# sp-uhh/sgmse

Measured on AMD Instinct MI355X. Metric: utterances/sec, SGMSE+ NCSN++ PC N=30 (reverse_diffusion + ALD, 60 NFE), 16 kHz 4 s utterances, higher is better.
Workload: dtype f32 (fp16x2-split products, fp32 accumulate); 1 GPU; BASELINE configs[1]: ncsnpp (65.6M params) PC sampler N=30, batch=32 x 4 s @16 kHz per GPU, hipGraph-captured step; batch_per_gpu=32, F=256, T=512, nfe=60, sampler=pc, parallelism=utterance-sharded x1 (weights broadcast once over RCCL)

## Files before the change

sgmse_amd/csrc/kernels_conv_split.h:

```cpp
#pragma once
#include "kernels_conv.h"

#ifndef SGMSE_SPLIT_FENCE
#define SGMSE_SPLIT_FENCE 0
#endif

namespace sgmse {

struct SplitB3 {
  static constexpr int NS = 3;
  static constexpr int NP = 6;
  static constexpr int PX_V = 7;
  static constexpr bool SCALED = false;
  __device__ static constexpr int pa(int k) { return k == 0 ? 2 : (k == 2 || k == 3) ? 1 : 0; }
  __device__ static constexpr int pb(int k) { return k == 1 ? 2 : (k == 2 || k == 4) ? 1 : 0; }
  __device__ static __forceinline__ void split(float x, uint32_t (&t)[3]) {
    const uint32_t xb = __builtin_bit_cast(uint32_t, x);
    const uint32_t hi = xb & 0xffff0000u;
    const float r1 = x - __builtin_bit_cast(float, hi);
    const uint32_t mid = __builtin_bit_cast(uint32_t, r1) & 0xffff0000u;
    const float r2 = r1 - __builtin_bit_cast(float, mid);
    t[0] = hi >> 16; t[1] = mid >> 16; t[2] = __builtin_bit_cast(uint32_t, r2) >> 16;
  }
  __device__ static __forceinline__ void split2(float x0, float x1, uint32_t (&d)[3]) {
    uint32_t a[3], b[3];
    split(x0, a); split(x1, b);
#pragma unroll
    for (int s = 0; s < 3; ++s) d[s] = a[s] | (b[s] << 16);
  }
  __device__ static __forceinline__ f32x16 mfma(u32x4 a, u32x4 b, f32x16 c) { return mfma_32x32x16_bf16(a, b, c); }
};

struct SplitH2 {
  static constexpr int NS = 2;
  static constexpr int NP = 3;
  static constexpr int PX_V = 5;
  static constexpr bool SCALED = true;
  __device__ static constexpr int pa(int k) { return k == 0 ? 1 : 0; }
  __device__ static constexpr int pb(int k) { return k == 1 ? 1 : 0; }
  __device__ static __forceinline__ void split(float x, uint32_t (&t)[2]) {
    const uint32_t hi = drt_f32_to_f16(x);
    const float r = x - drt_f16_to_f32(hi);
    t[0] = hi; t[1] = drt_f32_to_f16(r);
  }
  __device__ static __forceinline__ void split2(float x0, float x1, uint32_t (&d)[2]) {
    const uint32_t hi = drt_f32x2_to_f16x2(x0, x1);
    d[0] = hi; d[1] = drt_f32x2_to_f16x2(drt_sub_f16_lo(x0, hi), drt_sub_f16_hi(x1, hi));
  }
  __device__ static __forceinline__ f32x16 mfma(u32x4 a, u32x4 b, f32x16 c) { return mfma_32x32x16_f16(a, b, c); }
};

template <int ROWS_>
struct ConvSplitGeom {
  static constexpr int KC = 16, ROWS = ROWS_, TROWS = ROWS_ + 2, TCOLS = 34;
  static constexpr int NITEM = TROWS * TCOLS * 2;
  static constexpr int NIT = (NITEM + 255) / 256;
};

struct PackSplitArgs { const float* src; uint32_t* dst; int cin, cout; size_t total; const float* co_scale; int taps; };
__global__ __launch_bounds__(256) void split_co_scale_kernel(const float* src, int n_per_co, int cout, int cout_pad, float* inv_scale, float* scale) {
  const int co = blockIdx.x * 256 + threadIdx.x;
  if (co >= cout_pad) return;
  float m = 0.f;
  if (co < cout) for (int i = 0; i < n_per_co; ++i) m = fmaxf(m, fabsf(src[(size_t)co * n_per_co + i]));
  const float sc = co < cout ? h2_weight_scale(m) : 1.f;
  scale[co] = sc; inv_scale[co] = 1.f / sc;
}

__global__ __launch_bounds__(256) void absmax_kernel(const float* x, size_t n, float* out) {
  float m = 0.f;
  for (size_t i = (size_t)blockIdx.x * 256 + threadIdx.x; i < n; i += (size_t)gridDim.x * 256) m = fmaxf(m, fabsf(x[i]));
#pragma unroll
  for (int o = 32; o >= 1; o >>= 1) m = fmaxf(m, __shfl_xor(m, o));
  if ((threadIdx.x & 63) == 0) drt_atomic_max_nonneg(out, m);
}

template <class S>
__global__ __launch_bounds__(256) void pack_weights_split_kernel(PackSplitArgs p) {
  const size_t e = (size_t)blockIdx.x * 256 + threadIdx.x;
  if (e >= p.total) return;
  const int lane = (int)(e & 63);
  size_t r = e >> 6;
  const int w = (int)(r & 3); r >>= 2;
  const int split = (int)(r % S::NS); r /= S::NS;
  const int tap = (int)(r % p.taps); r /= p.taps;
  const int nst = p.cin / 16;
  const int st = (int)(r % nst);
  const int blk = (int)(r / nst);
  const int co = blk * 128 + w * 32 + (lane & 31);
  const int c0 = st * 16 + 8 * (lane >> 5);
  const float wscale = (S::SCALED && co < p.cout) ? p.co_scale[co] : 1.f;
  u32x4 o;
#pragma unroll
  for (int q = 0; q < 4; ++q) {
    uint32_t part[2];
#pragma unroll
    for (int h = 0; h < 2; ++h) {
      const int c = c0 + 2 * q + h;
      const float v = (co < p.cout ? p.src[((size_t)co * p.cin + c) * p.taps + tap] : 0.f) * wscale;
      uint32_t t[S::NS];
      S::split(v, t);
      uint32_t sel = t[0];
#pragma unroll
      for (int s = 1; s < S::NS; ++s) sel = split == s ? t[s] : sel;
      part[h] = sel;
    }
    o[q] = part[0] | (part[1] << 16);
  }
  reinterpret_cast<u32x4*>(p.dst)[e] = o;
}

template <class S>
inline size_t packed_split_frags(int cin, int cout, int taps = 9) { return (size_t)((cout + 127) / 128) * (cin / 16) * taps * S::NS * 4 * 64; }
template <class S>
inline size_t packed_split_bytes(int cin, int cout, int taps = 9) { return packed_split_frags<S>(cin, cout, taps) * 16 + (size_t)((cout + 127) / 128) * 128 * 8; }

template <class S, int SHAPE = 0, int ACT = 1, int ABL = 0, int SC = 0, int CHK = 0>
__global__ __launch_bounds__(256, 2) void conv3x3_split_kernel(ConvArgs p) {
  static_assert(!CHK || (SHAPE == 2 && !SC), "chunked accumulation exists for the plain 4-row shape");
  constexpr bool THIN = SHAPE == 1;
  constexpr int ROWS = SHAPE == 2 ? 4 : 8;
  using C = ConvSplitGeom<ROWS>;
  constexpr int WCW = THIN ? 1 : 4;
  constexpr int FCW = THIN ? 1 : 4 / WCW;
  constexpr int FPW = THIN ? 2 : ROWS / (4 / WCW);
  using T = ConvTile<3, WCW, FCW, FPW, 1>;
  static_assert(T::CO_T == (THIN ? 32 : 128) && T::ROWS == ROWS, "tile");
  constexpr int NS = S::NS, PX_V = S::PX_V;
  constexpr int EPJ = 8 / FPW;
  constexpr int STAGE_V = C::TROWS * C::TCOLS * PX_V;
  constexpr int DUMMY_V = STAGE_V;
  __shared__ u32x4 s_in0[STAGE_V + NS];
  __shared__ u32x4 s_in1[STAGE_V + NS];
  constexpr int NCO = S::SCALED ? 4 : 2;
  __shared__ float s_co[512 * NCO];

  const int tid = threadIdx.x;
  if constexpr (ABL & 512) {
    __shared__ u32x4 s_pad[3072];
    if (p.ablate == 12345) s_pad[tid] = u32x4{0u, 0u, 0u, 0u};
  }
  unsigned long long* trace = nullptr;
  if constexpr (ABL & 64) {
    if (tid == 0 && p.trace) {
      trace = p.trace + 16 * (size_t)(blockIdx.y * gridDim.x + blockIdx.x);
      trace[0] = (unsigned long long)drt_hw_id() | ((unsigned long long)drt_xcc_id() << 32);
      trace[1] = drt_clock();
    }
  }
  const int Cin = p.C1 + p.C2;
  const int tiles_xg = (p.W + 31) >> 5;
  const int tiles_y = (p.H + ROWS - 1) / ROWS;
  int b, ty, tx;
  conv_tile_of(p, (int)blockIdx.x, (int)gridDim.x, tiles_xg, tiles_y, b, ty, tx);
  if (p.rag_w) { if (!conv_ragged_adjust(p, b, tx)) return; }
  const int H = p.H, W = p.W;
  const int tiles_x = (W + 31) >> 5;
  const int co_blk = blockIdx.y;
  const int x0 = tx * 32, y0 = ty * ROWS;
  float xb_raw = 0.f;
  if constexpr (S::SCALED) { if (p.xbound) xb_raw = p.xbound[b * kAmaxSpread + (tid & (kAmaxSpread - 1))]; }
  float csc[2], csh[2];
#pragma unroll
  for (int k = 0; k < 2; ++k) {
    const int c = tid + 256 * k;
    const bool ld = p.in_scale != nullptr && c < Cin;
    csc[k] = ld ? p.in_scale[b * Cin + (c < Cin ? c : 0)] : 1.f;
    csh[k] = ld ? p.in_shift[b * Cin + (c < Cin ? c : 0)] : 0.f;
  }
  const unsigned HW = (unsigned)H * (unsigned)W;

  const int wave = tid >> 6, lane = tid & 63, l31 = lane & 31, kg = lane >> 5;

  unsigned it_boff[C::NIT];
  int it_loff[C::NIT], it_g[C::NIT];
#pragma unroll
  for (int i = 0; i < C::NIT; ++i) {
    int it = tid + 256 * i;
    it = it < C::NITEM ? it : C::NITEM - 1;
    const int g = it / (C::TROWS * C::TCOLS);
    const int rem = it - g * (C::TROWS * C::TCOLS);
    const int r = rem / C::TCOLS, c = rem - r * C::TCOLS;
    const int gy = y0 - 1 + r, gx = x0 - 1 + c;
    const bool ok = gy >= 0 && gy < H && gx >= 0 && gx < W;
    const int loff = (r * C::TCOLS + c) * PX_V + g * NS;
    if (!ok) {
#pragma unroll
      for (int s = 0; s < NS; ++s) { s_in0[loff + s] = u32x4{0u, 0u, 0u, 0u}; s_in1[loff + s] = u32x4{0u, 0u, 0u, 0u}; }
    }
    it_boff[i] = ((unsigned)(8 * g) * HW + (ok ? (unsigned)(gy * W + gx) : 0u)) * 4u;
    it_loff[i] = ok ? loff : DUMMY_V;
    it_g[i] = g;
  }

  float rin[C::NIT][8];
  auto load_item = [&](int i, int c0) {
    const bool first = c0 < p.C1;
    const float* base = first ? p.src1 + ((size_t)b * p.C1 + c0) * HW : p.src2 + ((size_t)b * p.C2 + (c0 - p.C1)) * HW;
#pragma unroll
    for (int e = 0; e < 8; ++e)
      rin[i][e] = *reinterpret_cast<const float*>(reinterpret_cast<const char*>(base + (size_t)e * HW) + it_boff[i]);
  };
  auto produce = [&](float x, int ch) -> float {
    float o, u;
    if constexpr (NCO == 4) {
      const f32x4 co = reinterpret_cast<const f32x4*>(s_co)[ch];
      o = x * co[0] + co[1];
      u = x * co[2] + co[3];
    } else {
      o = x * s_co[2 * ch] + s_co[2 * ch + 1];
      u = o * -1.4426950408889634f;
    }
    if constexpr (ACT == 1) {
      if constexpr (ABL & 4) o = o * u;
      else o = o * __builtin_amdgcn_rcpf(1.0f + drt_exp2(u));
    }
    if (S::SCALED) o = fminf(fmaxf(o, -65504.f), 65504.f);
    return o;
  };
  auto store_item = [&](int i, int c0, u32x4* sbuf) {
    u32x4 v[NS];
#pragma unroll
    for (int q = 0; q < 4; ++q) {
      const int ch = c0 + 8 * it_g[i] + 2 * q;
      uint32_t d[NS];
      S::split2(produce(rin[i][2 * q], ch), produce(rin[i][2 * q + 1], ch + 1), d);
#pragma unroll
      for (int s = 0; s < NS; ++s) v[s][q] = d[s];
    }
#pragma unroll
    for (int s = 0; s < NS; ++s) sbuf[it_loff[i] + s] = v[s];
  };

  u32x4 pk[NS];
  float ev = 0.f;
  auto stage_elem = [&](int i, int e, int c0, const float (&raw)[C::NIT][8]) {
    const float o = produce(raw[i][e], c0 + 8 * it_g[i] + e);
    if ((e & 1) == 0) { ev = o; return; }
    uint32_t d[NS];
    S::split2(ev, o, d);
#pragma unroll
    for (int s = 0; s < NS; ++s) pk[s][e >> 1] = d[s];
  };
  auto flush_item = [&](int i, u32x4* sbuf) {
#pragma unroll
    for (int s = 0; s < NS; ++s) sbuf[it_loff[i] + s] = pk[s];
  };

  const int wc = THIN ? 0 : wave % WCW, wp = THIN ? wave : wave / WCW;
  const int nst = Cin / C::KC;
  int st0 = 0, st1 = nst;
  if constexpr (CHK) {
    if (gridDim.z > 1) { st0 = (int)blockIdx.z * p.kchunk_stages; st1 = st0 + p.kchunk_stages < nst ? st0 + p.kchunk_stages : nst; }
  }
  float acc_raw[(SC || CHK) ? 1 : FCW][16];
  if constexpr (!(SC || CHK)) {
#pragma unroll
    for (int i = 0; i < FCW; ++i) conv_acc_raw<T>(p, b, co_blk, wc * FCW + i, kg, acc_raw[i]);
  }
  float sc_m1 = 0.f, sc_m2 = 0.f;
  if constexpr (SC) {
    sc_m1 = p.sc_amax1[b * kAmaxSpread + (tid & (kAmaxSpread - 1))];
    if (p.sc_amax2) sc_m2 = p.sc_amax2[b * kAmaxSpread + (tid & (kAmaxSpread - 1))];
  } else {
#pragma unroll
    for (int i = 0; i < C::NIT; ++i) load_item(i, st0 * C::KC);
  }
  float kx = 1.f;
  if constexpr (S::SCALED) {
    if (p.xbound) {
#pragma unroll
      for (int o = 32; o >= 1; o >>= 1) xb_raw = fmaxf(xb_raw, __shfl_xor(xb_raw, o));
      kx = h2_weight_scale(xb_raw);
    }
  }
  const float inv_kx = 1.f / kx;
  {
    constexpr float nl2e = -1.4426950408889634f;
#pragma unroll
    for (int k = 0; k < 2; ++k) {
      const int c = tid + 256 * k;
      if (c < Cin) {
        if constexpr (NCO == 4) {
          f32x4 v;
          v[0] = csc[k] * kx; v[1] = csh[k] * kx; v[2] = csc[k] * nl2e; v[3] = csh[k] * nl2e;
          reinterpret_cast<f32x4*>(s_co)[c] = v;
        } else {
          s_co[2 * c] = csc[k] * kx; s_co[2 * c + 1] = csh[k] * kx;
        }
      }
    }
  }
  f32x16 acc[FCW][FPW];
#pragma unroll
  for (int i = 0; i < FCW; ++i) {
    float init[16];
    if constexpr (SC || CHK) {
#pragma unroll
      for (int r = 0; r < 16; ++r) init[r] = 0.f;
    } else {
      const int co_l = co_blk * T::CO_T + (wc * FCW + i) * 32 + 4 * kg;
#pragma unroll
      for (int r = 0; r < 16; ++r) init[r] = acc_raw[i][r] * (1.0f / (conv_as(p, co_l + (r & 3) + 8 * (r >> 2)) * inv_kx));
    }
#pragma unroll
    for (int j = 0; j < FPW; ++j)
#pragma unroll
      for (int r = 0; r < 16; ++r) acc[i][j][r] = init[r];
  }

  const u32x4* wblk = reinterpret_cast<const u32x4*>(p.w) + (size_t)co_blk * nst * 9 * NS * 4 * 64;
  const unsigned a_boff = (unsigned)((wc * FCW * 64 + lane) * 16);
  const bool a_real = !THIN || l31 < p.Cout;
  auto load_a = [&](int st, int tap, u32x4 (&a)[FCW][NS]) {
    const u32x4* q = wblk + (size_t)(st * 9 + tap) * NS * 4 * 64;
#pragma unroll
    for (int i = 0; i < FCW; ++i)
#pragma unroll
      for (int s = 0; s < NS; ++s) {
        if constexpr (THIN) {
          a[i][s] = u32x4{0u, 0u, 0u, 0u};
          if (a_real) a[i][s] = *reinterpret_cast<const u32x4*>(reinterpret_cast<const char*>(q + s * 4 * 64 + i * 64) + a_boff);
        } else {
          a[i][s] = *reinterpret_cast<const u32x4*>(reinterpret_cast<const char*>(q + s * 4 * 64 + i * 64) + a_boff);
        }
      }
  };
  const int b_lane = l31 * PX_V + kg * NS + wp * FPW * C::TCOLS * PX_V;

  u32x4 bq[2][NS];
  auto compute_tap = [&](const u32x4* sbuf, int tap, const u32x4 (&a)[FCW][NS], int item, int c0n, u32x4* nxt, const float (&raw)[C::NIT][8]) {
    const int dy = tap / 3, dx = tap - 3 * dy;
    const u32x4* sb = sbuf + b_lane + (dy * C::TCOLS + dx) * PX_V;
    if constexpr (!(ABL & 16)) {
#pragma unroll
      for (int s = 0; s < NS; ++s) bq[0][s] = sb[s];
    }
#pragma unroll
    for (int j = 0; j < FPW; ++j) {
      if constexpr (!(ABL & 16)) {
        if (j + 1 < FPW) {
          const u32x4* q = sb + (j + 1) * C::TCOLS * PX_V;
#pragma unroll
          for (int s = 0; s < NS; ++s) bq[(j + 1) & 1][s] = q[s];
        }
      }
      __builtin_amdgcn_sched_barrier(SGMSE_SPLIT_FENCE);
#pragma unroll
      for (int k = 0; k < S::NP; ++k)
#pragma unroll
        for (int i = 0; i < FCW; ++i) acc[i][j] = S::mfma(a[i][S::pa(k)], bq[j & 1][S::pb(k)], acc[i][j]);
      if (item >= 0) {
#pragma unroll
        for (int e = 0; e < EPJ; ++e) stage_elem(item, j * EPJ + e, c0n, raw);
        if (j == FPW - 1) flush_item(item, nxt);
      }
      __builtin_amdgcn_sched_barrier(SGMSE_SPLIT_FENCE);
    }
  };

  if constexpr (SC) {
    static_assert(S::SCALED && !THIN, "the folded shortcut exists for the fp16x2 full-block shapes");
    float m = fmaxf(sc_m1, sc_m2);
#pragma unroll
    for (int o = 32; o >= 1; o >>= 1) m = fmaxf(m, __shfl_xor(m, o));
    const float xs = h2_weight_scale(m);
    const int nsts = (p.sc_C1 + p.sc_C2) / C::KC;
    float rsc[C::NIT][8];
    auto load_sc = [&](int c0, float (&dst)[C::NIT][8]) {
      const bool first = c0 < p.sc_C1;
      const float* base = first ? p.sc_src1 + ((size_t)b * p.sc_C1 + c0) * HW : p.sc_src2 + ((size_t)b * p.sc_C2 + (c0 - p.sc_C1)) * HW;
#pragma unroll
      for (int i = 0; i < C::NIT; ++i)
#pragma unroll
        for (int e = 0; e < 8; ++e)
          dst[i][e] = *reinterpret_cast<const float*>(reinterpret_cast<const char*>(base + (size_t)e * HW) + it_boff[i]);
    };
    auto store_sc = [&](const float (&src)[C::NIT][8], u32x4* sbuf) {
#pragma unroll
      for (int i = 0; i < C::NIT; ++i) {
        u32x4 v[NS];
#pragma unroll
        for (int q = 0; q < 4; ++q) {
          uint32_t d[NS];
          S::split2(fminf(fmaxf(src[i][2 * q] * xs, -65504.f), 65504.f), fminf(fmaxf(src[i][2 * q + 1] * xs, -65504.f), 65504.f), d);
#pragma unroll
          for (int s = 0; s < NS; ++s) v[s][q] = d[s];
        }
#pragma unroll
        for (int s = 0; s < NS; ++s) sbuf[it_loff[i] + s] = v[s];
      }
    };
    const u32x4* wsc = reinterpret_cast<const u32x4*>(p.sc_w) + (size_t)co_blk * nsts * NS * 4 * 64;
    auto load_asc = [&](int st, u32x4 (&a)[FCW][NS]) {
      const u32x4* q = wsc + (size_t)st * NS * 4 * 64;
#pragma unroll
      for (int i = 0; i < FCW; ++i)
#pragma unroll
        for (int s = 0; s < NS; ++s)
          a[i][s] = *reinterpret_cast<const u32x4*>(reinterpret_cast<const char*>(q + s * 4 * 64 + i * 64) + a_boff);
    };
    load_sc(0, rin);
    load_sc((nsts > 1 ? 1 : 0) * C::KC, rsc);
    __syncthreads();
    store_sc(rin, s_in0);
    __syncthreads();
    u32x4 asc[FCW][NS];
#pragma unroll 1
    for (int st = 0; st < nsts; st += 2) {
      load_asc(st, asc);
      if (st + 2 < nsts) load_sc((st + 2) * C::KC, rin);
      compute_tap(s_in0, 4, asc, -1, 0, s_in1, rin);
      if (st + 1 < nsts) store_sc(rsc, s_in1);
      __syncthreads();
      if (st + 1 < nsts) {
        load_asc(st + 1, asc);
        if (st + 3 < nsts) load_sc((st + 3) * C::KC, rsc);
        compute_tap(s_in1, 4, asc, -1, 0, s_in0, rin);
        if (st + 2 < nsts) store_sc(rin, s_in0);
        __syncthreads();
      }
    }
#pragma unroll
    for (int i = 0; i < FCW; ++i) {
      float init[16], rho[16];
      conv_acc_init<T>(p, b, co_blk, wc * FCW + i, kg, inv_kx, init);
      const int co_l = co_blk * T::CO_T + (wc * FCW + i) * 32 + 4 * kg;
#pragma unroll
      for (int r = 0; r < 16; ++r) {
        const int co = co_l + (r & 3) + 8 * (r >> 2);
        const float as3 = conv_as(p, co) * inv_kx;
        rho[r] = (p.sc_scale[co] / xs) / as3;
        init[r] += p.sc_bias ? p.sc_bias[co] / as3 : 0.f;
      }
#pragma unroll
      for (int j = 0; j < FPW; ++j)
#pragma unroll
        for (int r = 0; r < 16; ++r) acc[i][j][r] = acc[i][j][r] * rho[r] + init[r];
    }
  }
  if constexpr (SC) {
#pragma unroll
    for (int i = 0; i < C::NIT; ++i) load_item(i, st0 * C::KC);
  }
  __syncthreads();
#pragma unroll
  for (int i = 0; i < C::NIT; ++i) store_item(i, st0 * C::KC, s_in0);
  __syncthreads();

  if constexpr (ABL & 64) { if (trace) trace[2] = drt_clock(); }
  unsigned long long tsum[10] = {0, 0, 0, 0, 0, 0, 0, 0, 0, 0};
  if constexpr (THIN && !ABL) {
    static_assert(FCW == 1, "thin shape");
    float rin2[C::NIT][8];
    u32x4 af[9][FCW][NS];
#pragma unroll
    for (int t = 0; t < 9; ++t) load_a(0, t, af[t]);
    auto load_raw = [&](int i, int c0, float (&dst)[C::NIT][8]) {
      const bool first = c0 < p.C1;
      const float* base = first ? p.src1 + ((size_t)b * p.C1 + c0) * HW : p.src2 + ((size_t)b * p.C2 + (c0 - p.C1)) * HW;
#pragma unroll
      for (int e = 0; e < 8; ++e)
        dst[i][e] = *reinterpret_cast<const float*>(reinterpret_cast<const char*>(base + (size_t)e * HW) + it_boff[i]);
    };
    auto clampst = [&](int st) { return st < nst ? st : nst - 1; };
#pragma unroll
    for (int i = 0; i < C::NIT; ++i) { load_raw(i, clampst(1) * C::KC, rin); load_raw(i, clampst(2) * C::KC, rin2); }
    auto thin_stage = [&](int st, const u32x4* cur, u32x4* nxt, float (&raw)[C::NIT][8]) {
      const int stn = clampst(st + 1), str = clampst(st + 3);
#pragma unroll
      for (int tap = 0; tap < 9; ++tap) {
        const int item = (tap >= 4 && (tap & 1) == 0 && (tap - 4) / 2 < C::NIT) ? (tap - 4) / 2 : -1;
        compute_tap(cur, tap, af[tap], item, stn * C::KC, nxt, raw);
        load_a(stn, tap, af[tap]);
        if (item >= 0) load_raw(item, str * C::KC, raw);
        __builtin_amdgcn_sched_barrier(0);
      }
      __syncthreads();
    };
#pragma unroll 1
    for (int st = 0; st < nst; st += 2) {
      thin_stage(st, s_in0, s_in1, rin);
      if (st + 1 < nst) thin_stage(st + 1, s_in1, s_in0, rin2);
    }
    conv_epilogue<T, FCW, FPW, WCW, 0, true, false, S::SCALED>(p, acc, b, co_blk, tx, ty, tiles_x, wc, wp, l31, kg, inv_kx);
      return;
  }
  constexpr int AR = 3, AD = AR - 1;
  u32x4 ar[AR][FCW][NS];
#pragma unroll
  for (int t = 0; t < AD; ++t) load_a(st0, t, ar[t]);
  f32x16 tot[CHK ? FCW : 1][CHK ? FPW : 1];
  bool first_chunk = true;
  if constexpr (ABL & 16) {
#pragma unroll
    for (int s = 0; s < NS; ++s) { bq[0][s] = s_in0[b_lane + s]; bq[1][s] = s_in0[b_lane + C::TCOLS * PX_V + s]; }
  }
  if constexpr (ABL & 32) load_a(0, 2, ar[2]);
#pragma unroll 1
  for (int st = st0; st < st1; ++st) {
    const int stn = st + 1 < st1 ? st + 1 : st;
    const u32x4* cur = ((st - st0) & 1) ? s_in1 : s_in0;
    u32x4* nxt = ((st - st0) & 1) ? s_in0 : s_in1;
#pragma unroll
    for (int tap = 0; tap < 9; ++tap) {
      unsigned long long tc0 = 0;
      if constexpr (ABL & 64) tc0 = drt_clock();
      const int ntap = (tap + AD) % 9;
      const int nstg = tap + AD < 9 ? st : stn;
      if constexpr (!(ABL & 32)) load_a(nstg, ntap, ar[(tap + AD) % AR]);
      if constexpr (!(ABL & 8)) { if (tap < C::NIT) load_item(tap, stn * C::KC); }
      __builtin_amdgcn_sched_barrier(0);
      int item = (tap >= 4 && (tap & 1) == 0 && (tap - 4) / 2 < C::NIT) ? (tap - 4) / 2 : -1;
      if constexpr (ABL & 8) item = -1;
      compute_tap(cur, tap, ar[tap % AR], item, stn * C::KC, nxt, rin);
      if constexpr (ABL & 64) { __builtin_amdgcn_sched_barrier(0); tsum[tap] += drt_clock() - tc0; }
    }
    if constexpr (ABL & 64) {
      const unsigned long long tb = drt_clock();
      __syncthreads();
      tsum[9] += drt_clock() - tb;
    } else {
      __syncthreads();
    }
    if constexpr (CHK) {
      if (gridDim.z == 1 && ((st + 1) % p.kchunk_stages == 0 || st + 1 == st1)) {
#pragma unroll
        for (int i = 0; i < FCW; ++i)
#pragma unroll
          for (int j = 0; j < FPW; ++j)
#pragma unroll
            for (int r = 0; r < 16; ++r) { tot[i][j][r] = first_chunk ? acc[i][j][r] : tot[i][j][r] + acc[i][j][r]; acc[i][j][r] = 0.f; }
        first_chunk = false;
      }
    }
  }
  if constexpr (CHK) {
    if (gridDim.z == 1) {
#pragma unroll
      for (int i = 0; i < FCW; ++i)
#pragma unroll
        for (int j = 0; j < FPW; ++j) acc[i][j] = tot[i][j];
    } else {
      ConvArgs q = p;
      q.out = p.partial + (size_t)blockIdx.z * conv_partial_slab(p, H, W);
      q.bias = nullptr; q.bias2 = nullptr; q.res = nullptr; q.acc_scale = nullptr; q.co_scale = nullptr; q.out_scale = 1.f; q.stats_out = nullptr; q.amax_out = nullptr;
      conv_epilogue<T, FCW, FPW, WCW, 0, true>(q, acc, b, co_blk, tx, ty, tiles_x, wc, wp, l31, kg);
      return;
    }
  }
  if constexpr (ABL & 64) {
    if (trace) {
#pragma unroll
      for (int i = 0; i < 10; ++i) trace[5 + i] = tsum[i];
    }
  }

  if constexpr (ABL & 64) { if (trace) trace[3] = drt_clock(); }
  conv_epilogue<T, FCW, FPW, WCW, ABL & (3 | 128 | 256), !CHK, FPW % 4 == 0, S::SCALED>(p, acc, b, co_blk, tx, ty, tiles_x, wc, wp, l31, kg, inv_kx);
  if constexpr (ABL & 64) { if (trace) trace[4] = drt_clock(); }
}

template <class S, int XF = 1, int VEC = 0>
__global__ __launch_bounds__(256, 2) void conv1x1_split_kernel(ConvArgs p) {
  using T = ConvTile<1, 4, 1, 8, 1>;
  static_assert(T::CO_T == 128 && T::ROWS == 8, "tile");
  static_assert(!VEC || !XF, "16-byte staging exists for raw inputs only");
  constexpr int NS = S::NS, PX_V = S::PX_V, KC = 16, NIT = 2;
  constexpr int STAGE_V = 256 * PX_V;
  __shared__ u32x4 s_in0[STAGE_V];
  __shared__ u32x4 s_in1[STAGE_V];
  __shared__ float s_sc[XF ? 512 : 1];
  __shared__ float s_sh[XF ? 512 : 1];

  const int tid = threadIdx.x;
  const int Cin = p.C1 + p.C2;
  const int tiles_xg = (p.W + 31) >> 5;
  const int tiles_y = (p.H + 7) >> 3;
  int b, ty, tx;
  conv_tile_of(p, (int)blockIdx.x, (int)gridDim.x, tiles_xg, tiles_y, b, ty, tx);
  if (p.rag_w) { if (!conv_ragged_adjust(p, b, tx)) return; }
  const int H = p.H, W = p.W;
  const int tiles_x = (W + 31) >> 5;
  const int co_blk = blockIdx.y;
  const int x0 = tx * 32, y0 = ty * 8;
  float actf = 0.f;
  if constexpr (XF) {
    const bool xform = p.in_scale != nullptr;
    for (int c = tid; c < Cin; c += 256) {
      s_sc[c] = xform ? p.in_scale[b * Cin + c] : 1.f;
      s_sh[c] = xform ? p.in_shift[b * Cin + c] : 0.f;
    }
    actf = (xform && p.in_act) ? 1.f : 0.f;
  }
  const size_t HW = (size_t)H * W;
  const int wave = tid >> 6, lane = tid & 63, l31 = lane & 31, kg = lane >> 5;
  float xs = 1.f;
  if (S::SCALED) {
    float m = p.amax1 ? amax_read(p.amax1, b) : 0.f;
    if (p.amax2) m = fmaxf(m, amax_read(p.amax2, b));
    xs = h2_weight_scale(m);
  }

  int it_goff[NIT], it_loff[NIT], it_g[NIT];
  if constexpr (VEC) {
    const int cq = tid & 7, h = (tid >> 3) & 1, g = (tid >> 4) & 1, r = tid >> 5;
    int gy = y0 + r, gx = x0 + 4 * cq;
    gy = gy < H ? gy : H - 1; gx = gx < W ? gx : W - 4;
    it_goff[0] = gy * W + gx;
    it_loff[0] = ((r * 32 + 4 * cq) * PX_V + g * NS) * 2 + h;
    it_g[0] = 8 * g + 4 * h;
    it_goff[1] = it_loff[1] = it_g[1] = 0;
  } else {
#pragma unroll
    for (int i = 0; i < NIT; ++i) {
      const int it = tid + 256 * i;
      const int g = it >> 8, r = (it >> 5) & 7, c = it & 31;
      int gy = y0 + r, gx = x0 + c;
      gy = gy < H ? gy : H - 1; gx = gx < W ? gx : W - 1;
      it_goff[i] = gy * W + gx;
      it_loff[i] = (r * 32 + c) * PX_V + g * NS;
      it_g[i] = g;
    }
  }
  float rinA[NIT][8], rinB[NIT][8];
  auto load_items = [&](int c0, float (&dst)[NIT][8]) {
    const bool first = c0 < p.C1;
    const float* base = first ? p.src1 + ((size_t)b * p.C1 + c0) * HW : p.src2 + ((size_t)b * p.C2 + (c0 - p.C1)) * HW;
    if constexpr (VEC) {
#pragma unroll
      for (int e = 0; e < 4; ++e) {
        const f32x4 v = *reinterpret_cast<const f32x4*>(base + (size_t)(it_g[0] + e) * HW + it_goff[0]);
#pragma unroll
        for (int q = 0; q < 4; ++q) dst[e >> 1][4 * (e & 1) + q] = v[q];
      }
    } else {
#pragma unroll
      for (int i = 0; i < NIT; ++i)
#pragma unroll
        for (int e = 0; e < 8; ++e) dst[i][e] = base[(size_t)(8 * it_g[i] + e) * HW + it_goff[i]];
    }
  };
  u32x4 pk[NS];
  uint32_t ev[NS];
  auto stage_elem = [&](int i, int e, int c0, const float (&src)[NIT][8]) {
    float t = src[i][e];
    if constexpr (XF) {
      const int ch = c0 + 8 * it_g[i] + e;
      t = t * s_sc[ch] + s_sh[ch];
      const float sig = __builtin_amdgcn_rcpf(1.0f + __expf(-t));
      t *= actf * (sig - 1.0f) + 1.0f;
    }
    if (S::SCALED) t = fminf(fmaxf(t * xs, -65504.f), 65504.f);
    uint32_t t16[NS];
    S::split(t, t16);
#pragma unroll
    for (int s = 0; s < NS; ++s) {
      if ((e & 1) == 0) ev[s] = t16[s]; else pk[s][e >> 1] = ev[s] | (t16[s] << 16);
    }
  };
  auto flush_item = [&](int i, u32x4* sbuf) {
#pragma unroll
    for (int s = 0; s < NS; ++s) sbuf[it_loff[i] + s] = pk[s];
  };
  uint32_t hv[NS];
  auto stage_quad = [&](int k, const float (&src)[NIT][8], u32x4* sbuf) {
    const int q = k >> 1, cp = k & 1;
    float t0 = src[cp][q], t1 = src[cp][4 + q];
    if (S::SCALED) { t0 = fminf(fmaxf(t0 * xs, -65504.f), 65504.f); t1 = fminf(fmaxf(t1 * xs, -65504.f), 65504.f); }
    uint32_t d[NS];
    S::split2(t0, t1, d);
    if (cp == 0) {
#pragma unroll
      for (int s = 0; s < NS; ++s) hv[s] = d[s];
    } else {
      typedef unsigned long long __attribute__((may_alias)) u64a;
      u64a* q8 = reinterpret_cast<u64a*>(sbuf) + it_loff[0] + q * PX_V * 2;
#pragma unroll
      for (int s = 0; s < NS; ++s) q8[2 * s] = (unsigned long long)hv[s] | ((unsigned long long)d[s] << 32);
    }
  };

  f32x16 acc[1][8];
#pragma unroll
  for (int j = 0; j < 8; ++j)
#pragma unroll
    for (int r = 0; r < 16; ++r) acc[0][j][r] = 0.f;

  const int nst = Cin / KC;
  const u32x4* wbase = reinterpret_cast<const u32x4*>(p.w) + (size_t)co_blk * nst * NS * 4 * 64 + wave * 64 + lane;
  auto load_a = [&](int st, u32x4 (&a)[NS]) {
    const u32x4* q = wbase + (size_t)st * NS * 4 * 64;
#pragma unroll
    for (int s = 0; s < NS; ++s) a[s] = q[s * 4 * 64];
  };
  const int b_lane = l31 * PX_V + kg * NS;

  load_items(0, rinA);
  if constexpr (XF) __syncthreads();
  if constexpr (VEC) {
#pragma unroll
    for (int k = 0; k < 8; ++k) stage_quad(k, rinA, s_in0);
  } else {
#pragma unroll
    for (int i = 0; i < NIT; ++i) {
#pragma unroll
      for (int e = 0; e < 8; ++e) stage_elem(i, e, 0, rinA);
      flush_item(i, s_in0);
    }
  }
  load_items((nst > 1 ? 1 : 0) * KC, rinA);
  u32x4 a0[NS], a1[NS];
  load_a(0, a0);
  __syncthreads();

#pragma unroll 1
  for (int st = 0; st < nst; ++st) {
    const int st1 = st + 1 < nst ? st + 1 : st, st2 = st + 2 < nst ? st + 2 : nst - 1;
    const u32x4* cur = (st & 1) ? s_in1 : s_in0;
    u32x4* nxt = (st & 1) ? s_in0 : s_in1;
    load_a(st1, a1);
    load_items(st2 * KC, rinB);
    __builtin_amdgcn_sched_barrier(0);
    const u32x4* sb = cur + b_lane;
    u32x4 bq[2][NS];
#pragma unroll
    for (int s = 0; s < NS; ++s) bq[0][s] = sb[s];
#pragma unroll
    for (int j = 0; j < 8; ++j) {
      if (j + 1 < 8) {
        const u32x4* q = sb + (j + 1) * 32 * PX_V;
#pragma unroll
        for (int s = 0; s < NS; ++s) bq[(j + 1) & 1][s] = q[s];
      }
      __builtin_amdgcn_sched_barrier(0);
      f32x16 c = acc[0][j];
#pragma unroll
      for (int k = 0; k < S::NP; ++k) c = S::mfma(a0[S::pa(k)], bq[j & 1][S::pb(k)], c);
      acc[0][j] = c;
      if constexpr (VEC) {
        stage_quad(j, rinA, nxt);
      } else {
        stage_elem(j >> 2, 2 * (j & 3), st1 * KC, rinA);
        stage_elem(j >> 2, 2 * (j & 3) + 1, st1 * KC, rinA);
        if ((j & 3) == 3) flush_item(j >> 2, nxt);
      }
      __builtin_amdgcn_sched_barrier(0);
    }
    __syncthreads();
#pragma unroll
    for (int s = 0; s < NS; ++s) a0[s] = a1[s];
#pragma unroll
    for (int i = 0; i < NIT; ++i)
#pragma unroll
      for (int e = 0; e < 8; ++e) rinA[i][e] = rinB[i][e];
  }

  conv_epilogue<T, 1, 8, 4, 0, false, true, S::SCALED>(p, acc, b, co_blk, tx, ty, tiles_x, wave, 0, l31, kg, 1.0f / xs);
}

}
```

Before: 6.210 utterances/s.

## Add three-deep register ring prefetch and bank-swap staging to conv1x1 split kernel

For the vectorized conv1x1 split path, global input loads are issued three stages ahead through a ring of register sets, and the MFMA loop is interleaved with staging of the next stage into shared memory using sched barriers. For NS==2 splits, the two packed 64-bit shared stores are swapped on alternating lane groups, apparently to spread LDS bank conflicts. This hides global load latency behind compute at the cost of more VGPRs, with a possible occupancy loss or spill risk (the static_assert notes that a ring of four spills).

```diff
diff --git a/sgmse_amd/csrc/kernels_conv_split.h b/sgmse_amd/csrc/kernels_conv_split.h
--- a/sgmse_amd/csrc/kernels_conv_split.h
+++ b/sgmse_amd/csrc/kernels_conv_split.h
@@ -561,11 +561,20 @@
   if constexpr (ABL & 64) { if (trace) trace[4] = drt_clock(); }
 }
 
+#ifndef SGMSE_CONV1X1_RING
+#define SGMSE_CONV1X1_RING 3
+#endif
+#ifndef SGMSE_CONV1X1_SWAP
+#define SGMSE_CONV1X1_SWAP 1
+#endif
 template <class S, int XF = 1, int VEC = 0>
 __global__ __launch_bounds__(256, 2) void conv1x1_split_kernel(ConvArgs p) {
   using T = ConvTile<1, 4, 1, 8, 1>;
   static_assert(T::CO_T == 128 && T::ROWS == 8, "tile");
   static_assert(!VEC || !XF, "16-byte staging exists for raw inputs only");
+  constexpr int RING = VEC ? SGMSE_CONV1X1_RING : 0;
+  static_assert(RING == 0 || RING == 3, "ring of raw-value register sets (a ring of four spills: 948 bytes of scratch per lane)");
+  constexpr bool SWAP = VEC && SGMSE_CONV1X1_SWAP && S::NS == 2;
   constexpr int NS = S::NS, PX_V = S::PX_V, KC = 16, NIT = 2;
   constexpr int STAGE_V = 256 * PX_V;
   __shared__ u32x4 s_in0[STAGE_V];
@@ -610,7 +619,8 @@
     it_goff[0] = gy * W + gx;
     it_loff[0] = ((r * 32 + 4 * cq) * PX_V + g * NS) * 2 + h;
     it_g[0] = 8 * g + 4 * h;
-    it_goff[1] = it_loff[1] = it_g[1] = 0;
+    it_goff[1] = it_g[1] = 0;
+    it_loff[1] = SWAP ? (cq >> 2) & 1 : 0;
   } else {
 #pragma unroll
     for (int i = 0; i < NIT; ++i) {
@@ -676,8 +686,16 @@
     } else {
       typedef unsigned long long __attribute__((may_alias)) u64a;
       u64a* q8 = reinterpret_cast<u64a*>(sbuf) + it_loff[0] + q * PX_V * 2;
-#pragma unroll
-      for (int s = 0; s < NS; ++s) q8[2 * s] = (unsigned long long)hv[s] | ((unsigned long long)d[s] << 32);
+      if constexpr (SWAP) {
+        const unsigned long long v0 = (unsigned long long)hv[0] | ((unsigned long long)d[0] << 32);
+        const unsigned long long v1 = (unsigned long long)hv[NS - 1] | ((unsigned long long)d[NS - 1] << 32);
+        const int sw = it_loff[1];
+        q8[2 * sw] = sw ? v1 : v0;
+        q8[2 - 2 * sw] = sw ? v0 : v1;
+      } else {
+#pragma unroll
+        for (int s = 0; s < NS; ++s) q8[2 * s] = (unsigned long long)hv[s] | ((unsigned long long)d[s] << 32);
+      }
     }
   };
 
@@ -695,6 +713,58 @@
     for (int s = 0; s < NS; ++s) a[s] = q[s * 4 * 64];
   };
   const int b_lane = l31 * PX_V + kg * NS;
+
+  if constexpr (RING != 0) {
+    constexpr int U = 2 * RING;
+    float rin[RING][NIT][8];
+    u32x4 af[2][NS];
+    auto clamped = [&](int s) { return s < nst ? s : nst - 1; };
+    load_items(0, rin[0]);
+#pragma unroll
+    for (int k = 1; k < RING - 1; ++k) load_items(clamped(k) * KC, rin[k]);
+    load_a(0, af[0]);
+    load_items(clamped(RING - 1) * KC, rin[RING - 1]);
+#pragma unroll
+    for (int k = 0; k < 8; ++k) stage_quad(k, rin[0], s_in0);
+    __syncthreads();
+    auto stage_body = [&](int st, const float (&use)[NIT][8], float (&ld)[NIT][8], const u32x4 (&a_cur)[NS], u32x4 (&a_nxt)[NS]) {
+      const u32x4* cur = (st & 1) ? s_in1 : s_in0;
+      u32x4* nxt = (st & 1) ? s_in0 : s_in1;
+      load_a(clamped(st + 1), a_nxt);
+      load_items(clamped(st + RING) * KC, ld);
+      __builtin_amdgcn_sched_barrier(0);
+      const u32x4* sb = cur + b_lane;
+      u32x4 bq[2][NS];
+#pragma unroll
+      for (int s = 0; s < NS; ++s) bq[0][s] = sb[s];
+#pragma unroll
+      for (int j = 0; j < 8; ++j) {
+        if (j + 1 < 8) {
+          const u32x4* q = sb + (j + 1) * 32 * PX_V;
+#pragma unroll
+          for (int s = 0; s < NS; ++s) bq[(j + 1) & 1][s] = q[s];
+        }
+        __builtin_amdgcn_sched_barrier(0);
+        f32x16 c = acc[0][j];
+#pragma unroll
+        for (int k = 0; k < S::NP; ++k) c = S::mfma(a_cur[S::pa(k)], bq[j & 1][S::pb(k)], c);
+        acc[0][j] = c;
+        stage_quad(j, use, nxt);
+        __builtin_amdgcn_sched_barrier(0);
+      }
+      __syncthreads();
+    };
+#pragma unroll 1
+    for (int st0 = 0; st0 < nst; st0 += U) {
+#pragma unroll
+      for (int u = 0; u < U; ++u) {
+        if (st0 + u >= nst) break;
+        stage_body(st0 + u, rin[(u + 1) % RING], rin[u % RING], af[u & 1], af[(u + 1) & 1]);
+      }
+    }
+    conv_epilogue<T, 1, 8, 4, 0, false, true, S::SCALED>(p, acc, b, co_blk, tx, ty, tiles_x, wave, 0, l31, kg, 1.0f / xs);
+    return;
+  }
 
   load_items(0, rinA);
   if constexpr (XF) __syncthreads();
```

New measurement: 6.212 utterances/s, median of 6. No clear change (+0.0%).
